# weleen/AGRL.pytorch

Hardware: NVIDIA B200
Metric: MARS-shape tracklets/s (graph head) + query×gallery eval ms at 1/2/4/8 B200 (higher is better)
Workload: dtype fp32 (head GEMMs: fp16 + e4m3 correction planes, distance: fp16x2 planes / 3 products, on tcgen05; fp32 accumulate)

## Files before the change

agrl/pytorch_b200/csrc/gemm_sm100.cuh:

```cuda
#pragma once
#include <cuda.h>
#include <cuda_bf16.h>

#include "common.cuh"

namespace agrl {
namespace gemm {

constexpr int BM = 128, BK = 64;
constexpr int UMMA_K = 16;
constexpr int kTileBytesA = BM * BK * 2;
constexpr int kCtrlWarps = 4;
constexpr int kAccStages = 2;
constexpr int kTmemCols = 512;
constexpr int kEpiPad = 33;
constexpr int kEpiBytes = 4 * 32 * kEpiPad * 4;

template <int P, int BN, bool kSplit, bool kDirect = false, int kChunkKb = 0, bool kPair = false> struct Config {
    static_assert(kChunkKb == 0 || (!kDirect && BN == 128), "chunked accumulation: 128-wide tiles, smem-transposed stores");
    static constexpr int kEpiWarps = (kDirect || kChunkKb > 0) ? 8 : 4;
    static constexpr int kThreads = 32 * (kCtrlWarps + kEpiWarps);
    static_assert(BN == 128 || BN == 256, "tile width");
    static_assert(!kSplit || BN == 128, "two accumulators of 256 columns do not fit twice in TMEM");
    static constexpr int kLoadN = kPair ? BN / 2 : BN;
// ... 39 lines not shown
__device__ __forceinline__ void mbar_wait(uint32_t bar, uint32_t parity) {
    asm volatile(
        "{\n\t"
        ".reg .pred p;\n\t"
        "WAIT_LOOP:\n\t"
        "mbarrier.try_wait.parity.shared::cta.b64 p, [%0], %1;\n\t"
        "@p bra WAIT_DONE;\n\t"
        "bra WAIT_LOOP;\n\t"
        "WAIT_DONE:\n\t"
        "}" ::"r"(bar), "r"(parity) : "memory");
}
__device__ __forceinline__ void tma_load_3d(uint32_t dst, const CUtensorMap *map, uint32_t bar, int c0, int c1, int c2) {
    asm volatile(
        "cp.async.bulk.tensor.3d.shared::cluster.global.mbarrier::complete_tx::bytes [%0], [%1, {%3, %4, %5}], [%2];"
        ::"r"(dst), "l"(reinterpret_cast<uint64_t>(map)), "r"(bar), "r"(c0), "r"(c1), "r"(c2) : "memory");
}
__device__ __forceinline__ void prefetch_tensormap(const CUtensorMap *map) {
    asm volatile("prefetch.tensormap [%0];" ::"l"(reinterpret_cast<uint64_t>(map)) : "memory");
}
__device__ __forceinline__ void tmem_alloc(uint32_t dst_smem, uint32_t ncols) {
    asm volatile("tcgen05.alloc.cta_group::1.sync.aligned.shared::cta.b32 [%0], %1;" ::"r"(dst_smem), "r"(ncols) : "memory");
}
__device__ __forceinline__ void tmem_relinquish() {
    asm volatile("tcgen05.relinquish_alloc_permit.cta_group::1.sync.aligned;" ::: "memory");
}
__device__ __forceinline__ void tmem_dealloc(uint32_t taddr, uint32_t ncols) {
    asm volatile("tcgen05.dealloc.cta_group::1.sync.aligned.b32 %0, %1;" ::"r"(taddr), "r"(ncols) : "memory");
}
__device__ __forceinline__ void tc_fence_before() { asm volatile("tcgen05.fence::before_thread_sync;" ::: "memory"); }
__device__ __forceinline__ void tc_fence_after() { asm volatile("tcgen05.fence::after_thread_sync;" ::: "memory"); }
// ... 597 lines not shown
                  int M, int N, int k_pad, Epi epi) {
    split_gemm_body<P, BN, kSplit, Epi>(map_a, map_b, M, N, k_pad, epi);
}

template <int P, int BN, bool kSplit, class Epi>
__global__ void __cluster_dims__(2, 1, 1) __maxnreg__((Config<P, BN, kSplit, Epi::kDirect, Epi::kChunkKb>::kMaxRegs))
pair_gemm_kernel(const __grid_constant__ CUtensorMap map_a, const __grid_constant__ CUtensorMap map_b,
                 int M, int N, int k_pad, Epi epi) {
    split_gemm_body<P, BN, kSplit, Epi, true>(map_a, map_b, M, N, k_pad, epi);
}

int make_plane_tensor_map(CUtensorMap *map, const void *planes, int64_t rows, int64_t k_pad, int P, int box_rows,
                          int64_t plane_rows);

int make_rows_tensor_map_f32(CUtensorMap *map, const float *x, int64_t batch, int V, int C, int box_channels);

template <int P, int BN, bool kSplit, class Epi>
int launch_pair_gemm(const CUtensorMap &map_a, const CUtensorMap &map_b, int M, int N, int k_pad, const Epi &epi, cudaStream_t st) {
    using Cfg = Config<P, BN, kSplit, Epi::kDirect, Epi::kChunkKb, true>;
    static_assert(!Epi::kDirect || !kSplit, "the direct epilogue reads a single accumulator");
    auto kern = pair_gemm_kernel<P, BN, kSplit, Epi>;
    AGRL_CUDA_TRY(cudaFuncSetAttribute(kern, cudaFuncAttributeMaxDynamicSharedMemorySize, Cfg::kSmemBytes));
    static const int max_pairs = [&] {
        cudaLaunchConfig_t cfg = {};
        cfg.gridDim = dim3(kNumSMs & ~1); cfg.blockDim = dim3(Cfg::kThreads); cfg.dynamicSmemBytes = Cfg::kSmemBytes;
        cudaLaunchAttribute at;
        at.id = cudaLaunchAttributeClusterDimension;
        at.val.clusterDim.x = 2; at.val.clusterDim.y = 1; at.val.clusterDim.z = 1;
        cfg.attrs = &at; cfg.numAttrs = 1;
        int n = 0;
// ... 46 lines not shown
```

agrl/pytorch_b200/csrc/head.cu:

```cuda
#include "gemm_sm100.cuh"

#include <cuda_fp16.h>
#include <cuda_fp8.h>

namespace agrl {

constexpr int kParts = 7;
constexpr int kMaxNodes = 64;
constexpr int kHeadThreads = 256;

static inline int planes_of(int split) { return split == AGRL_SPLIT_FP16_E4M3 ? 2 : split; }
static inline bool scaled_mode(int split) { return split == AGRL_SPLIT_FP16X1 || split == AGRL_SPLIT_FP16_E4M3; }

struct FoldArgs {
    const float *w[AGRL_HEAD_MAX_LAYERS + 2], *b[AGRL_HEAD_MAX_LAYERS + 2];
    const float *mean[AGRL_HEAD_MAX_LAYERS + 2], *var[AGRL_HEAD_MAX_LAYERS + 2];
    float *scale[AGRL_HEAD_MAX_LAYERS + 2], *shift[AGRL_HEAD_MAX_LAYERS + 2];
    int channels;
    float eps;
};

__global__ void fold_bn_kernel(FoldArgs a) {
    const int which = blockIdx.y;
    for (int c = blockIdx.x * blockDim.x + threadIdx.x; c < a.channels; c += gridDim.x * blockDim.x) {
// ... 61 lines not shown
    static __device__ __forceinline__ float cvt(__half v) { return __half2float(v); }
    static __device__ __forceinline__ float4 cvt4(const uint2 &v) {
        const float2 lo = __half22float2(*reinterpret_cast<const __half2 *>(&v.x));
        const float2 hi = __half22float2(*reinterpret_cast<const __half2 *>(&v.y));
        return make_float4(lo.x, lo.y, hi.x, hi.y);
    }
};

template <class T>
struct PoolArgs {
    const T *x41, *x42;
    float *nodes;
    float *out; int64_t ld_out;
    const float *g_scale, *g_shift;
    int S, C, hw;
};

constexpr int kPoolCh = 64;

template <bool kVec, class T>
__global__ void __launch_bounds__(kHeadThreads)
pool_kernel(PoolArgs<T> a) {
    using E = MapElem<T>;
    using Vec4 = typename E::Vec4;
    extern __shared__ float s_nodes[];
    const int b = blockIdx.y, c0 = blockIdx.x * kPoolCh;
    const int warp = threadIdx.x >> 5, lane = threadIdx.x & 31;
    const int grp = lane >> 3, sub = lane & 7;
    const int hw = a.hw, qlen = hw >> 2;
    const float inv_q = 1.0f / static_cast<float>(qlen), inv_h = 1.0f / static_cast<float>(2 * qlen);
// ... 38 lines not shown
            float *dst = s_nodes + (s * kParts) * kPoolCh + warp * 8 + i;
            if (sub == 0) dst[grp * kPoolCh] = v2 * inv_q;
            if (lane == 0) { dst[4 * kPoolCh] = h2 * inv_h; dst[6 * kPoolCh] = w2 * inv_w; }
            if (lane == 16) dst[5 * kPoolCh] = h2 * inv_h;
        }
    }
    if (lane == 0) {
        const float inv_all = 1.0f / (static_cast<float>(a.S) * static_cast<float>(hw));
#pragma unroll
        for (int i = 0; i < 8; ++i) {
            const int c = c0 + warp * 8 + i;
            a.out[static_cast<size_t>(b) * a.ld_out + c] = fmaf(gsum[i] * inv_all, a.g_scale[c], a.g_shift[c]);
        }
    }
    __syncthreads();
    const int V = a.S * kParts;
    float *nodes = a.nodes + static_cast<size_t>(b) * V * a.C + c0;
    for (int i = threadIdx.x; i < V * kPoolCh; i += kHeadThreads) {
        const int v = i / kPoolCh, c = i % kPoolCh;
        nodes[static_cast<size_t>(v) * a.C + c] = s_nodes[i];
    }
}

__device__ __forceinline__ void add4(float4 &a, const float4 &b) { a.x += b.x; a.y += b.y; a.z += b.z; a.w += b.w; }
__device__ __forceinline__ float4 scale4(const float4 &a, float s) { return make_float4(a.x * s, a.y * s, a.z * s, a.w * s); }

template <class T>
__global__ void __launch_bounds__(kHeadThreads)
pool_nhwc_kernel(PoolArgs<T> a) {
    using E = MapElem<T>;
    using Vec4 = typename E::Vec4;
    const int b = blockIdx.y;
    const int c = (blockIdx.x * kHeadThreads + threadIdx.x) * 4;
    if (c >= a.C) return;
    const int hw = a.hw, qlen = hw >> 2, V = a.S * kParts;
// ... 11 lines not shown
#pragma unroll 8
            for (int p = 0; p < qlen; ++p) {
                add4(s1, E::cvt4(__ldcs(reinterpret_cast<const Vec4 *>(a.x41 + base + static_cast<size_t>(p) * a.C))));
                add4(s2, E::cvt4(__ldcs(reinterpret_cast<const Vec4 *>(a.x42 + base + static_cast<size_t>(p) * a.C))));
            }
            add4(g, s1);
            q[k] = s2;
        }
        float4 h0 = q[0], h1 = q[2];
        add4(h0, q[1]); add4(h1, q[3]);
        float4 w = h0;
        add4(w, h1);
        float *row = nodes + static_cast<size_t>(s) * kParts * a.C;
#pragma unroll
        for (int k = 0; k < 4; ++k) *reinterpret_cast<float4 *>(row + static_cast<size_t>(k) * a.C) = scale4(q[k], inv_q);
        *reinterpret_cast<float4 *>(row + 4 * static_cast<size_t>(a.C)) = scale4(h0, inv_h);
        *reinterpret_cast<float4 *>(row + 5 * static_cast<size_t>(a.C)) = scale4(h1, inv_h);
        *reinterpret_cast<float4 *>(row + 6 * static_cast<size_t>(a.C)) = scale4(w, inv_w);
    }
    const float inv_all = 1.0f / (static_cast<float>(a.S) * static_cast<float>(hw));
    const float4 sc = *reinterpret_cast<const float4 *>(a.g_scale + c), sh = *reinterpret_cast<const float4 *>(a.g_shift + c);
    float4 o;
    o.x = fmaf(g.x * inv_all, sc.x, sh.x); o.y = fmaf(g.y * inv_all, sc.y, sh.y);
    o.z = fmaf(g.z * inv_all, sc.z, sh.z); o.w = fmaf(g.w * inv_all, sc.w, sh.w);
    float *dst = a.out + static_cast<size_t>(b) * a.ld_out + c;
    dst[0] = o.x; dst[1] = o.y; dst[2] = o.z; dst[3] = o.w;
}

constexpr int kTpCh = 32;
constexpr int kTpConsumerWarps = 4;
constexpr int kTpThreads = 32 * (1 + kTpConsumerWarps);
template <class T> constexpr int tp_stage_bytes() { return kTpCh * 128 * static_cast<int>(sizeof(T)); }
template <class T> constexpr int tp_default_stages() { return sizeof(T) == 4 ? 4 : 12; }

template <class T>
struct PoolTmaArgs {
    const T *x41, *x42;
    float *nodes;
    float *out; int64_t ld_out;
    const float *g_scale, *g_shift;
    int S, C, stages;
    int unit0, unit1;
    int l2_hint;
};

static size_t pool_tma_smem(int S, int stages, int stage_bytes) {
    const size_t b = static_cast<size_t>(stages) * stage_bytes + 2 * static_cast<size_t>(S) * kParts * kTpCh * sizeof(float) +
                     2 * static_cast<size_t>(stages) * 8;
    return ((b + 127) & ~static_cast<size_t>(127)) + 128;
}

__device__ __forceinline__ void bulk_load_evict_first(uint32_t dst, const void *src, uint32_t bytes, uint32_t bar,
                                                      uint64_t policy) {
    asm volatile(
        "cp.async.bulk.shared::cluster.global.mbarrier::complete_tx::bytes.L2::cache_hint [%0], [%1], %2, [%3], %4;"
        ::"r"(dst), "l"(src), "r"(bytes), "r"(bar), "l"(policy) : "memory");
}

// ... 57 lines not shown
                for (int s = 0; s < S; ++s) {
                    const size_t off = ((static_cast<size_t>(b) * S + s) * C + static_cast<size_t>(cc) * kTpCh) * 128;
#pragma unroll
                    for (int m = 0; m < 2; ++m) {
                        gemm::mbar_wait(bar_empty + 8 * stage, phase ^ 1);
                        const uint32_t full = bar_full + 8 * stage;
                        gemm::mbar_arrive_expect_tx(full, kStageBytes);
                        if (a.l2_hint) bulk_load_evict_first(ring + stage * kStageBytes, (m ? a.x42 : a.x41) + off, kStageBytes, full, policy);
                        else bulk_load(ring + stage * kStageBytes, (m ? a.x42 : a.x41) + off, kStageBytes, full);
                        if (++stage == stages) { stage = 0; phase ^= 1; }
                    }
                }
            }
        }
    } else {
        const int cw = warp - 1, ct = tid - 32;
        const int grp = lane >> 3, sub = lane & 7;
        const float inv_all = 1.0f / (static_cast<float>(S) * 128.0f);
        int stage = 0; uint32_t phase = 0; int it = 0;
        for (int u = first; u < units; u += stride, ++it) {
            const int b = u / chunks, c0 = (u % chunks) * kTpCh;
            float *sn = s_nodes + (it & 1) * V * kTpCh;
            float gsum[8];
#pragma unroll
            for (int i = 0; i < 8; ++i) gsum[i] = 0.f;
            for (int s = 0; s < S; ++s) {
                gemm::mbar_wait(bar_full + 8 * stage, phase);
                {
                    const Vec4 *p = ring_v + stage * kStageVec4 + (cw * 8) * 32 + lane;
#pragma unroll
                    for (int i = 0; i < 8; ++i) {
// ... 26 lines not shown
                    if (grp == 0) dst[6 * kTpCh] = w2 * (1.0f / 128.0f);
                }
                if (++stage == stages) { stage = 0; phase ^= 1; }
            }
            {
                float t = group8_transpose_sum(gsum, sub);
                t += __shfl_xor_sync(0xffffffffu, t, 8);
                t += __shfl_xor_sync(0xffffffffu, t, 16);
                if (grp == 0) {
                    const int c = c0 + cw * 8 + sub;
                    a.out[static_cast<size_t>(b) * a.ld_out + c] = fmaf(t * inv_all, a.g_scale[c], a.g_shift[c]);
                }
            }
            asm volatile("bar.sync 1, %0;" ::"n"(32 * kTpConsumerWarps) : "memory");
            float *nodes = a.nodes + static_cast<size_t>(b) * V * C + c0;
            for (int v = ct >> 5; v < V; v += kTpConsumerWarps) nodes[static_cast<size_t>(v) * C + lane] = sn[v * kTpCh + lane];
        }
    }
}



constexpr int kChunk = 128;
constexpr int kGLd = kMaxNodes + 4;

struct GraphArgs {
    const float *x;
    const float *adj;
    const uint64_t *masks;
    __nv_bfloat16 *y_planes;
    int64_t plane_stride;
// ... 19 lines not shown
        if (adj) return adj[r * V + c];
        const uint64_t hit = ((m0 >> r) & (m0 >> c)) | ((m1 >> r) & (m1 >> c)) | ((m2 >> r) & (m2 >> c));
        return (r != c && (hit & 1ull)) ? 1.0f : 0.0f;
    }
};

constexpr int kTcPlane = 64 * 128;
constexpr int kTcGPlanes = 0;
constexpr int kTcRingOff = 2 * kTcPlane;
constexpr int kTcRingBytes = 8 * kTcPlane;
constexpr int kTcBars = kTcRingOff + kTcRingBytes;
constexpr int kTcRawOff = kTcBars + 256;
constexpr int kTcSmem = kTcRawOff + 1024;
constexpr int kTcThreads = 448;
static_assert((kMaxNodes * kGLd + kMaxNodes) * 4 <= kTcRingBytes, "g[] fits the ring");

__device__ __forceinline__ void fence_proxy_async_smem() { asm volatile("fence.proxy.async.shared::cta;" ::: "memory"); }

template <int P>
__device__ __forceinline__ void split8(const float (&v)[8], uint4 (&out)[P]) {
    float r[8];
#pragma unroll
    for (int i = 0; i < 8; ++i) r[i] = v[i];
#pragma unroll
    for (int p = 0; p < P; ++p) {
        uint32_t w[4];
#pragma unroll
        for (int i = 0; i < 4; ++i) {
            const __nv_bfloat162 b = __floats2bfloat162_rn(r[2 * i], r[2 * i + 1]);
            w[i] = *reinterpret_cast<const uint32_t *>(&b);
// ... 64 lines not shown
            gemm::mbar_init(b_gfull + 8 * i, 8); gemm::mbar_init(b_gdone + 8 * i, 1);
        }
        gemm::fence_barrier_init();
    }
    if (warp == 0) { gemm::tmem_alloc(gemm::smem_u32(tmem_slot), 256); gemm::tmem_relinquish(); }
    if (!a.learn_graph && gram_worker) for (int i = tid; i < kMaxNodes * kGLd; i += kHeadThreads) g[i] = 0.f;
    gemm::tc_fence_before();
    __syncthreads();
    gemm::tc_fence_after();
    const uint32_t tmem = *tmem_slot;
    const bool epi_warp = gram_worker && (warp & 3) < 2;
    const int erow = (warp & 3) * 32 + lane, ehalf = warp >> 2;
    const uint32_t tlane = tmem + (static_cast<uint32_t>((warp & 3) * 32) << 16);
    auto wait_bar = [&](uint32_t bar, int use) { gemm::mbar_wait(bar, static_cast<uint32_t>(use & 1)); };
    const int ref_row = (V > 6) ? 6 : V - 1;
    const int n_gblocks = C / 64;
    if (warp == 0) AGRL_TL(0);
    const int raw_stage = V * 256;
    auto stage_off = [&](int st) { return st < 2 ? kTcRawOff + st * raw_stage : kTcRingOff + 6 * kTcPlane; };
    auto load_raw = [&](int piece, int st) {
        if (lane == 0) {
            const uint32_t full = b_rfull + 8 * st;
            gemm::mbar_arrive_expect_tx(full, static_cast<uint32_t>(raw_stage));
            gemm::tma_load_3d(gemm::smem_u32(smem) + stage_off(st), &map_x, full, piece * 64, 0, b);
        }
    };
    auto gram_uses_of = [&](int st) { return a.learn_graph ? (n_gblocks + 2 - st) / 3 : 0; };
    if (loader && lane == 0) gemm::prefetch_tensormap(&map_x);

    if (a.learn_graph) {
        if (gram_worker) {
            for (int kb = 0; kb < n_gblocks; ++kb) {
                const int buf = kb % 3, use = kb / 3;
                wait_bar(b_rfull + 8 * buf, use);
                if (warp == 0) AGRL_TL(96 + kb);
                if (kb >= 3) wait_bar(b_gdone + 8 * buf, use - 1);
                if (warp == 0) AGRL_TL(192 + kb);
                const float *rs = reinterpret_cast<const float *>(smem + stage_off(buf));
                const float4 *rsrc = reinterpret_cast<const float4 *>(rs + ref_row * 64 + (tid & 7) * 8);
                const float4 rlo = rsrc[0], rhi = rsrc[1];
                unsigned char *dst = ring_p + buf * 2 * kTcPlane;
#pragma unroll
                for (int t = 0; t < 2; ++t) {
                    const int item = tid + kHeadThreads * t, row = item >> 3, slot = item & 7;
                    float c[8];
                    if (row < V) {
                        const float4 *src = reinterpret_cast<const float4 *>(rs + row * 64 + slot * 8);
                        const float4 lo = src[0], hi = src[1];
                        c[0] = __fsub_rn(lo.x, rlo.x); c[1] = __fsub_rn(lo.y, rlo.y); c[2] = __fsub_rn(lo.z, rlo.z); c[3] = __fsub_rn(lo.w, rlo.w);
                        c[4] = __fsub_rn(hi.x, rhi.x); c[5] = __fsub_rn(hi.y, rhi.y); c[6] = __fsub_rn(hi.z, rhi.z); c[7] = __fsub_rn(hi.w, rhi.w);
                    } else {
#pragma unroll
                        for (int i = 0; i < 8; ++i) c[i] = 0.f;
                    }
                    uint4 pl[2];
                    split8<2>(c, pl);
                    const int off = row * 128 + ((slot ^ (row & 7)) << 4);
#pragma unroll
                    for (int p = 0; p < 2; ++p) *reinterpret_cast<uint4 *>(dst + p * kTcPlane + off) = pl[p];
                }
                fence_proxy_async_smem();
                __syncwarp();
                if (lane == 0) { gemm::mbar_arrive(b_gfull + 8 * buf); gemm::mbar_arrive(b_rempty + 8 * buf); }
// ... 73 lines not shown
                m1 = __fdiv_rn(__fdiv_rn(a1, ra) + __fdiv_rn(s1, rs), 2.0f);
            } else if (a.learn_graph) { m0 = __fdiv_rn(s0, rs); m1 = __fdiv_rn(s1, rs); }
            else { m0 = __fdiv_rn(a0, ra); m1 = __fdiv_rn(a1, ra); }
            __syncwarp();
            g[r * kGLd + lane] = (lane < V) ? m0 : 0.f;
            g[r * kGLd + c1] = (c1 < V) ? m1 : 0.f;
        }
    }
    __syncthreads();
    __shared__ float s_scale[2];
    float y_scale = 1.0f;
    if (a.fp16) {
        if (!a.learn_graph) {
            if (worker) {
                for (int r = warp; r < V; r += 12) {
                    const float4 *row = reinterpret_cast<const float4 *>(x + static_cast<size_t>(r) * C);
                    float t = 0.f;
                    for (int i = lane; i < C / 4; i += 32) {
                        const float4 v = __ldg(row + i);
                        t = fmaf(v.x, v.x, t); t = fmaf(v.y, v.y, t); t = fmaf(v.z, v.z, t); t = fmaf(v.w, v.w, t);
                    }
                    t = warp_sum(t);
                    if (lane == 0) sq[r] = t;
                }
            }
            __syncthreads();
        }
        if (warp == 0) {
            float m = fmaxf(lane < V ? sq[lane] : 0.f, lane + 32 < V ? sq[lane + 32] : 0.f);
#pragma unroll
            for (int o = 16; o > 0; o >>= 1) m = fmaxf(m, __shfl_xor_sync(0xffffffffu, m, o));
            float refn = 0.f;
            if (a.learn_graph) {
                const float4 *row = reinterpret_cast<const float4 *>(x + static_cast<size_t>(ref_row) * C);
                for (int i = lane; i < C / 4; i += 32) {
                    const float4 v = __ldg(row + i);
                    refn = fmaf(v.x, v.x, refn); refn = fmaf(v.y, v.y, refn); refn = fmaf(v.z, v.z, refn); refn = fmaf(v.w, v.w, refn);
                }
                refn = warp_sum(refn);
            }
            if (lane == 0) {
                m = (m < 3.0e38f && refn < 3.0e38f) ? sqrtf(m) + sqrtf(refn) : 0.f;
                pow2_scales(m, &s_scale[0], &s_scale[1]);
                a.y_unscale[b] = s_scale[1];
            }
        }
        __syncthreads();
        y_scale = s_scale[0];
    }
    if (a.lowrank) {
        if (worker) {
            const int S4 = (V / kParts) * 4;
            float *gt = a.gt + static_cast<size_t>(b) * V * S4;
            for (int i = tid; i < V * S4; i += 32 * 12) {
                const int r = i / S4, j = i - r * S4, k = j & 3;
                const float *gr = g + r * kGLd + (j >> 2) * kParts;
                gt[i] = fmaf(0.25f, gr[6], fmaf(0.5f, gr[4 + (k >> 1)], gr[k]));
            }
            const int groups = C / 8;
            for (int i = tid; i < S4 * groups; i += 32 * 12) {
                const int qr = i / groups, cg = i - qr * groups;
                const int row = (qr >> 2) * kParts + (qr & 3);
                const float4 *src = reinterpret_cast<const float4 *>(x + static_cast<size_t>(row) * C + cg * 8);
                const float4 lo = __ldg(src), hi = __ldg(src + 1);
                const float v[8] = {lo.x, lo.y, lo.z, lo.w, hi.x, hi.y, hi.z, hi.w};
                __nv_bfloat16 *dst = a.y_planes + (static_cast<size_t>(b) * S4 + qr) * C + cg * 8;
                if (a.fp8) {
// ... 191 lines not shown
    if (warp == 0) AGRL_TL(3);
    gemm::tc_fence_before();
    __syncthreads();
    if (warp == 0) gemm::tmem_dealloc(tmem, 256);
}

constexpr int kMixLdMax = 36;
struct MixArgs {
    const float *x, *z, *gt;
    float *out;
    const float *scale, *shift;
    int V, S4, C;
    float gamma, slope;
};

constexpr int kMixRows = 8;
template <int kMixLd>
__global__ void __launch_bounds__(kHeadThreads, 2)
graph_mix_kernel(MixArgs a) {
    __shared__ __align__(16) float s_gt[kMaxNodes * kMixLd];
    const int b = blockIdx.y, c = (blockIdx.x * kHeadThreads + threadIdx.x) * 2;
    const int V = a.V, S4 = a.S4, C = a.C;
    const float *gt = a.gt + static_cast<size_t>(b) * V * S4;
    for (int i = threadIdx.x; i < V * kMixLd; i += kHeadThreads) {
        const int r = i / kMixLd, k = i - r * kMixLd;
        s_gt[i] = (k < S4) ? gt[r * S4 + k] : 0.f;
    }
    float2 z[kMixLd];
    const float *zc = a.z + static_cast<size_t>(b) * S4 * C + c;
#pragma unroll
    for (int k = 0; k < kMixLd; ++k)
        z[k] = (k < S4) ? __ldg(reinterpret_cast<const float2 *>(zc + static_cast<size_t>(k) * C)) : make_float2(0.f, 0.f);
    const float2 sc = __ldg(reinterpret_cast<const float2 *>(a.scale + c)), sh = __ldg(reinterpret_cast<const float2 *>(a.shift + c));
    const float keep = 1.0f - a.gamma;
    const float *xc = a.x + static_cast<size_t>(b) * V * C + c;
    float *oc = a.out + static_cast<size_t>(b) * V * C + c;
    __syncthreads();
    for (int r0 = 0; r0 < V; r0 += kMixRows) {
        float2 xin[kMixRows];
#pragma unroll
        for (int i = 0; i < kMixRows; ++i)
            xin[i] = (r0 + i < V) ? __ldg(reinterpret_cast<const float2 *>(xc + static_cast<size_t>(r0 + i) * C)) : make_float2(0.f, 0.f);
#pragma unroll
        for (int i = 0; i < kMixRows; ++i) {
            if (r0 + i < V) {
                const float4 *g4 = reinterpret_cast<const float4 *>(s_gt + (r0 + i) * kMixLd);
                float a0 = 0.f, a1 = 0.f;
#pragma unroll
                for (int k4 = 0; k4 < kMixLd / 4; ++k4) {
                    const float4 w = g4[k4];
                    a0 = fmaf(w.x, z[4 * k4 + 0].x, a0); a1 = fmaf(w.x, z[4 * k4 + 0].y, a1);
                    a0 = fmaf(w.y, z[4 * k4 + 1].x, a0); a1 = fmaf(w.y, z[4 * k4 + 1].y, a1);
                    a0 = fmaf(w.z, z[4 * k4 + 2].x, a0); a1 = fmaf(w.z, z[4 * k4 + 2].y, a1);
                    a0 = fmaf(w.w, z[4 * k4 + 3].x, a0); a1 = fmaf(w.w, z[4 * k4 + 3].y, a1);
                }
                float h0 = fmaf(a0, sc.x, sh.x), h1 = fmaf(a1, sc.y, sh.y);
                h0 = h0 >= 0.f ? h0 : h0 * a.slope;
                h1 = h1 >= 0.f ? h1 : h1 * a.slope;
                float2 o;
                o.x = fmaf(a.gamma, h0, keep * xin[i].x);
                o.y = fmaf(a.gamma, h1, keep * xin[i].y);
                *reinterpret_cast<float2 *>(oc + static_cast<size_t>(r0 + i) * C) = o;
            }
        }
    }
}

struct AttnArgs {
    const float *x;
    float *out; int64_t ld_out;
    const float *a_scale, *a_shift;
    int S, C;
    const float *row_sumsq;
    int slots;
};

__global__ void __launch_bounds__(kHeadThreads)
attn_kernel(AttnArgs a) {
// ... 89 lines not shown
    if (!p) return AGRL_E_INVALID;
    if (p->num_layers < 0 || p->num_layers > AGRL_HEAD_MAX_LAYERS) return AGRL_E_INVALID;
    if (p->split != AGRL_SPLIT_BF16X2 && p->split != AGRL_SPLIT_BF16X3 && p->split != AGRL_SPLIT_FP16X1 &&
        p->split != AGRL_SPLIT_FP16_E4M3) return AGRL_E_INVALID;
    if (p->channels < kChunk || p->channels % kChunk != 0) return AGRL_E_UNSUPPORTED;
    if (!p->use_pose && !p->learn_graph) return AGRL_E_INVALID;
    if (p->pool_stages != 0 && (p->pool_stages < 2 || p->pool_stages > 12)) return AGRL_E_INVALID;
    if (p->maps_dtype != AGRL_MAPS_FP32 && p->maps_dtype != AGRL_MAPS_BF16 && p->maps_dtype != AGRL_MAPS_FP16) return AGRL_E_INVALID;
    return AGRL_OK;
}

static int launch_graph(const GraphArgs &ga, int64_t batch, cudaStream_t st) {
    const int smem = kTcSmem + 2 * ga.V * 256;
    AGRL_CUDA_TRY(cudaFuncSetAttribute(graph_kernel_tc, cudaFuncAttributeMaxDynamicSharedMemorySize, kTcSmem + 2 * kMaxNodes * 256));
    CUtensorMap map_x;
    int rc = gemm::make_rows_tensor_map_f32(&map_x, ga.x, batch, ga.V, ga.C, 64);
    if (rc) return rc;
    graph_kernel_tc<<<static_cast<unsigned>(batch), kTcThreads, smem, st>>>(map_x, ga);
    AGRL_LAUNCH_CHECK(st, "graph");
    return AGRL_OK;
}

}

using namespace agrl;

#ifdef AGRL_TIMELINE
extern "C" __attribute__((visibility("default"))) int agrl_timeline_set(long long *buf) {
    return cudaMemcpyToSymbol(g_timeline, &buf, sizeof(buf)) == cudaSuccess ? 0 : -3;
}
#endif
// ... 42 lines not shown
    return AGRL_OK;
}

extern "C" size_t agrl_head_workspace_bytes(const agrl_head_params *p, int64_t batch, int32_t seq_len) {
    if (check_params(p) || batch < 0 || seq_len < 1) return 0;
    return carve_head(p, nullptr, batch, seq_len).bytes;
}

namespace agrl {

template <class T>
static int launch_pool(const agrl_head_params *p, const Prepared &pr, const HeadWorkspace &hwk, const T *x4_1,
                       const T *x4_2, float *out, int64_t ld_out, int64_t b0, int64_t n, int S, int hw, bool tma,
                       cudaStream_t st) {
    const int C = p->channels, V = S * kParts, L = p->num_layers;
    const size_t in_off = static_cast<size_t>(b0) * S * C * hw;
    float *nodes = hwk.x[0] + static_cast<size_t>(b0) * V * C;
    float *o = out + static_cast<size_t>(b0) * ld_out;
    AGRL_LAUNCH_BEGIN(st);
    if (p->maps_nhwc) {
        PoolArgs<T> pa{x4_1 + in_off, x4_2 + in_off, nodes, o, ld_out, pr.scale[L], pr.shift[L], S, C, hw};
        const dim3 grid((C / 4 + kHeadThreads - 1) / kHeadThreads, static_cast<unsigned>(n));
        pool_nhwc_kernel<T><<<grid, kHeadThreads, 0, st>>>(pa);
        AGRL_LAUNCH_CHECK(st, "pool");
        return AGRL_OK;
    }
    if (tma) {
        const int64_t units = n * (C / kTpCh);
        PoolTmaArgs<T> ta{x4_1 + in_off, x4_2 + in_off, nodes, o, ld_out, pr.scale[L], pr.shift[L], S, C,
                          p->pool_stages ? p->pool_stages : tp_default_stages<T>(), 0, static_cast<int>(units),
                          p->pool_no_l2_hint ? 0 : 1};
        const size_t smem = pool_tma_smem(S, ta.stages, tp_stage_bytes<T>());
        AGRL_CUDA_TRY(cudaFuncSetAttribute(pool_tma_kernel<T>, cudaFuncAttributeMaxDynamicSharedMemorySize, static_cast<int>(smem)));
        int64_t grid = static_cast<int64_t>(kNumSMs) * 2;
        if (grid > units) grid = units;
        pool_tma_kernel<T><<<static_cast<unsigned>(grid), kTpThreads, smem, st>>>(ta);
        AGRL_LAUNCH_CHECK(st, "pool");
        return AGRL_OK;
    }
    PoolArgs<T> pa{x4_1 + in_off, x4_2 + in_off, nodes, o, ld_out, pr.scale[L], pr.shift[L], S, C, hw};
    const size_t pool_smem = static_cast<size_t>(S) * kParts * kPoolCh * sizeof(float);
    const dim3 pgrid(C / kPoolCh, static_cast<unsigned>(n));
    const uintptr_t vec_align = 4 * sizeof(T) - 1;
    const bool vec = (hw == 128) && ((reinterpret_cast<uintptr_t>(x4_1) | reinterpret_cast<uintptr_t>(x4_2)) & vec_align) == 0;
    if (vec) pool_kernel<true, T><<<pgrid, kHeadThreads, pool_smem, st>>>(pa);
    else pool_kernel<false, T><<<pgrid, kHeadThreads, pool_smem, st>>>(pa);
    AGRL_LAUNCH_CHECK(st, "pool");
    return AGRL_OK;
}

static int launch_pool_any(const agrl_head_params *p, const Prepared &pr, const HeadWorkspace &hwk, const void *x4_1,
                           const void *x4_2, float *out, int64_t ld_out, int64_t b0, int64_t n, int S, int hw, bool tma,
                           cudaStream_t st) {
    switch (p->maps_dtype) {
        case AGRL_MAPS_BF16:
// ... 191 lines not shown
```

agrl/pytorch_b200/csrc/split.cu:

```cuda
#include "gemm_sm100.cuh"

#include <cuda_fp16.h>
#include <cuda_fp8.h>
#include <mutex>

namespace agrl {
namespace gemm {

constexpr int kSplitThreads = 256;

__global__ void __launch_bounds__(kSplitThreads)
split_planes_kernel(SplitArgs a) {
    __shared__ float s_part[kSplitThreads / 32], s_maxp[kSplitThreads / 32];
    __shared__ float s_inv, s_ps;
    const int64_t row = blockIdx.x;
    const int tid = threadIdx.x;
    const float *src = a.src + row * a.ld;
    const bool vec = ((reinterpret_cast<uintptr_t>(src) & 15u) == 0) && (a.dim % 4 == 0);

    float inv = 1.0f, ps = 1.0f;
    if (a.sumsq != nullptr || a.normalize || a.fp16x2) {
        float s = 0.f, m = 0.f;
        if (vec) {
            const float4 *s4 = reinterpret_cast<const float4 *>(src);
// ... 124 lines not shown
    if (!fn) return AGRL_E_NO_DEVICE;
    const cuuint64_t dims[3] = {static_cast<cuuint64_t>(C), static_cast<cuuint64_t>(V), static_cast<cuuint64_t>(batch)};
    const cuuint64_t strides[2] = {static_cast<cuuint64_t>(C) * 4, static_cast<cuuint64_t>(V) * C * 4};
    const cuuint32_t box[3] = {static_cast<cuuint32_t>(box_channels), static_cast<cuuint32_t>(V), 1};
    const cuuint32_t estr[3] = {1, 1, 1};
    const CUresult r = fn(map, CU_TENSOR_MAP_DATA_TYPE_FLOAT32, 3, const_cast<float *>(x), dims, strides, box, estr,
                          CU_TENSOR_MAP_INTERLEAVE_NONE, CU_TENSOR_MAP_SWIZZLE_NONE,
                          CU_TENSOR_MAP_L2_PROMOTION_L2_256B, CU_TENSOR_MAP_FLOAT_OOB_FILL_NONE);
    if (r != CUDA_SUCCESS) {
        set_cuda_error(cudaErrorInvalidValue, "cuTensorMapEncodeTiled", __FILE__, __LINE__);
        return AGRL_E_CUDA;
    }
    return AGRL_OK;
}

}
}
```

Baseline: 203,200.

## Store only quarter-part nodes and rebuild half/whole parts on the fly

When the low-rank graph path is on, the pooling kernels write only the four quarter-part node rows per frame. The graph and mix kernels rebuild the two half-part rows and the whole-part row as means of the quarters when they need them. The graph kernel loads just the quarter rows through a new 4D TMA map, which cuts the raw staging bytes. It also folds the reference-row norm into the gram-worker loop instead of re-reading it from global memory. This trades pooled-node stores and global reads for a few extra adds, and relies on the half and whole poolings being exact means of the quarters in fp32 rounding order.

```diff
diff --git a/agrl/pytorch_b200/csrc/gemm_sm100.cuh b/agrl/pytorch_b200/csrc/gemm_sm100.cuh
--- a/agrl/pytorch_b200/csrc/gemm_sm100.cuh
+++ b/agrl/pytorch_b200/csrc/gemm_sm100.cuh
@@ -77,6 +77,11 @@
     asm volatile(
         "cp.async.bulk.tensor.3d.shared::cluster.global.mbarrier::complete_tx::bytes [%0], [%1, {%3, %4, %5}], [%2];"
         ::"r"(dst), "l"(reinterpret_cast<uint64_t>(map)), "r"(bar), "r"(c0), "r"(c1), "r"(c2) : "memory");
+}
+__device__ __forceinline__ void tma_load_4d(uint32_t dst, const CUtensorMap *map, uint32_t bar, int c0, int c1, int c2, int c3) {
+    asm volatile(
+        "cp.async.bulk.tensor.4d.shared::cluster.global.mbarrier::complete_tx::bytes [%0], [%1, {%3, %4, %5, %6}], [%2];"
+        ::"r"(dst), "l"(reinterpret_cast<uint64_t>(map)), "r"(bar), "r"(c0), "r"(c1), "r"(c2), "r"(c3) : "memory");
 }
 __device__ __forceinline__ void prefetch_tensormap(const CUtensorMap *map) {
     asm volatile("prefetch.tensormap [%0];" ::"l"(reinterpret_cast<uint64_t>(map)) : "memory");
@@ -704,6 +709,7 @@
                           int64_t plane_rows);
 
 int make_rows_tensor_map_f32(CUtensorMap *map, const float *x, int64_t batch, int V, int C, int box_channels);
+int make_quarter_rows_tensor_map_f32(CUtensorMap *map, const float *x, int64_t batch, int S, int C, int box_channels);
 
 template <int P, int BN, bool kSplit, class Epi>
 int launch_pair_gemm(const CUtensorMap &map_a, const CUtensorMap &map_b, int M, int N, int k_pad, const Epi &epi, cudaStream_t st) {
diff --git a/agrl/pytorch_b200/csrc/head.cu b/agrl/pytorch_b200/csrc/head.cu
--- a/agrl/pytorch_b200/csrc/head.cu
+++ b/agrl/pytorch_b200/csrc/head.cu
@@ -99,6 +99,7 @@
     float *out; int64_t ld_out;
     const float *g_scale, *g_shift;
     int S, C, hw;
+    int quarters_only;
 };
 
 constexpr int kPoolCh = 64;
@@ -167,11 +168,12 @@
         }
     }
     __syncthreads();
-    const int V = a.S * kParts;
+    const int V = a.S * kParts, R = a.quarters_only ? 4 * a.S : V;
     float *nodes = a.nodes + static_cast<size_t>(b) * V * a.C + c0;
-    for (int i = threadIdx.x; i < V * kPoolCh; i += kHeadThreads) {
-        const int v = i / kPoolCh, c = i % kPoolCh;
-        nodes[static_cast<size_t>(v) * a.C + c] = s_nodes[i];
+    for (int i = threadIdx.x; i < R * kPoolCh; i += kHeadThreads) {
+        const int r = i / kPoolCh, c = i % kPoolCh;
+        const int v = a.quarters_only ? (r >> 2) * kParts + (r & 3) : r;
+        nodes[static_cast<size_t>(v) * a.C + c] = s_nodes[v * kPoolCh + c];
     }
 }
 
@@ -213,6 +215,7 @@
         float *row = nodes + static_cast<size_t>(s) * kParts * a.C;
 #pragma unroll
         for (int k = 0; k < 4; ++k) *reinterpret_cast<float4 *>(row + static_cast<size_t>(k) * a.C) = scale4(q[k], inv_q);
+        if (a.quarters_only) continue;
         *reinterpret_cast<float4 *>(row + 4 * static_cast<size_t>(a.C)) = scale4(h0, inv_h);
         *reinterpret_cast<float4 *>(row + 5 * static_cast<size_t>(a.C)) = scale4(h1, inv_h);
         *reinterpret_cast<float4 *>(row + 6 * static_cast<size_t>(a.C)) = scale4(w, inv_w);
@@ -241,6 +244,7 @@
     int S, C, stages;
     int unit0, unit1;
     int l2_hint;
+    int quarters_only;
 };
 
 static size_t pool_tma_smem(int S, int stages, int stage_bytes) {
@@ -328,7 +332,7 @@
             }
         }
     } else {
-        const int cw = warp - 1, ct = tid - 32;
+        const int cw = warp - 1;
         const int grp = lane >> 3, sub = lane & 7;
         const float inv_all = 1.0f / (static_cast<float>(S) * 128.0f);
         int stage = 0; uint32_t phase = 0; int it = 0;
@@ -385,7 +389,8 @@
             }
             asm volatile("bar.sync 1, %0;" ::"n"(32 * kTpConsumerWarps) : "memory");
             float *nodes = a.nodes + static_cast<size_t>(b) * V * C + c0;
-            for (int v = ct >> 5; v < V; v += kTpConsumerWarps) nodes[static_cast<size_t>(v) * C + lane] = sn[v * kTpCh + lane];
+            const int vstep = a.quarters_only ? kParts : kTpConsumerWarps;
+            for (int v = cw; v < V; v += vstep) nodes[static_cast<size_t>(v) * C + lane] = sn[v * kTpCh + lane];
         }
     }
 }
@@ -435,6 +440,14 @@
 constexpr int kTcSmem = kTcRawOff + 1024;
 constexpr int kTcThreads = 448;
 static_assert((kMaxNodes * kGLd + kMaxNodes) * 4 <= kTcRingBytes, "g[] fits the ring");
+
+__device__ __forceinline__ float4 half_mean(const float4 &a, const float4 &b) {
+    return make_float4((a.x + b.x) * 0.5f, (a.y + b.y) * 0.5f, (a.z + b.z) * 0.5f, (a.w + b.w) * 0.5f);
+}
+__device__ __forceinline__ float4 quarter_mean(const float4 &a, const float4 &b, const float4 &c, const float4 &d) {
+    return make_float4(((a.x + b.x) + (c.x + d.x)) * 0.25f, ((a.y + b.y) + (c.y + d.y)) * 0.25f,
+                       ((a.z + b.z) + (c.z + d.z)) * 0.25f, ((a.w + b.w) + (c.w + d.w)) * 0.25f);
+}
 
 __device__ __forceinline__ void fence_proxy_async_smem() { asm volatile("fence.proxy.async.shared::cta;" ::: "memory"); }
 
@@ -529,20 +542,23 @@
     const uint32_t tlane = tmem + (static_cast<uint32_t>((warp & 3) * 32) << 16);
     auto wait_bar = [&](uint32_t bar, int use) { gemm::mbar_wait(bar, static_cast<uint32_t>(use & 1)); };
     const int ref_row = (V > 6) ? 6 : V - 1;
+    const int S4 = (V / kParts) * 4;
     const int n_gblocks = C / 64;
     if (warp == 0) AGRL_TL(0);
-    const int raw_stage = V * 256;
+    const int raw_stage = (a.lowrank ? S4 : V) * 256;
     auto stage_off = [&](int st) { return st < 2 ? kTcRawOff + st * raw_stage : kTcRingOff + 6 * kTcPlane; };
     auto load_raw = [&](int piece, int st) {
         if (lane == 0) {
             const uint32_t full = b_rfull + 8 * st;
             gemm::mbar_arrive_expect_tx(full, static_cast<uint32_t>(raw_stage));
-            gemm::tma_load_3d(gemm::smem_u32(smem) + stage_off(st), &map_x, full, piece * 64, 0, b);
+            if (a.lowrank) gemm::tma_load_4d(gemm::smem_u32(smem) + stage_off(st), &map_x, full, piece * 64, 0, 0, b);
+            else gemm::tma_load_3d(gemm::smem_u32(smem) + stage_off(st), &map_x, full, piece * 64, 0, b);
         }
     };
     auto gram_uses_of = [&](int st) { return a.learn_graph ? (n_gblocks + 2 - st) / 3 : 0; };
     if (loader && lane == 0) gemm::prefetch_tensormap(&map_x);
 
+    float refn_part = 0.f;
     if (a.learn_graph) {
         if (gram_worker) {
             for (int kb = 0; kb < n_gblocks; ++kb) {
@@ -552,16 +568,50 @@
                 if (kb >= 3) wait_bar(b_gdone + 8 * buf, use - 1);
                 if (warp == 0) AGRL_TL(192 + kb);
                 const float *rs = reinterpret_cast<const float *>(smem + stage_off(buf));
-                const float4 *rsrc = reinterpret_cast<const float4 *>(rs + ref_row * 64 + (tid & 7) * 8);
-                const float4 rlo = rsrc[0], rhi = rsrc[1];
+                float4 rlo, rhi;
+                if (a.lowrank) {
+                    const float4 *q = reinterpret_cast<const float4 *>(rs + (lane >> 3) * 64 + (tid & 7) * 8);
+                    rlo = q[0]; rhi = q[1];
+                    float *rv[8] = {&rlo.x, &rlo.y, &rlo.z, &rlo.w, &rhi.x, &rhi.y, &rhi.z, &rhi.w};
+#pragma unroll
+                    for (int i = 0; i < 8; ++i) {
+                        float v = *rv[i];
+                        v += __shfl_xor_sync(0xffffffffu, v, 8);
+                        v += __shfl_xor_sync(0xffffffffu, v, 16);
+                        *rv[i] = v * 0.25f;
+                    }
+                } else {
+                    const float4 *rsrc = reinterpret_cast<const float4 *>(rs + ref_row * 64 + (tid & 7) * 8);
+                    rlo = rsrc[0]; rhi = rsrc[1];
+                }
+                if (tid < 8) {
+                    refn_part = fmaf(rlo.x, rlo.x, refn_part); refn_part = fmaf(rlo.y, rlo.y, refn_part);
+                    refn_part = fmaf(rlo.z, rlo.z, refn_part); refn_part = fmaf(rlo.w, rlo.w, refn_part);
+                    refn_part = fmaf(rhi.x, rhi.x, refn_part); refn_part = fmaf(rhi.y, rhi.y, refn_part);
+                    refn_part = fmaf(rhi.z, rhi.z, refn_part); refn_part = fmaf(rhi.w, rhi.w, refn_part);
+                }
                 unsigned char *dst = ring_p + buf * 2 * kTcPlane;
 #pragma unroll
                 for (int t = 0; t < 2; ++t) {
                     const int item = tid + kHeadThreads * t, row = item >> 3, slot = item & 7;
                     float c[8];
                     if (row < V) {
-                        const float4 *src = reinterpret_cast<const float4 *>(rs + row * 64 + slot * 8);
-                        const float4 lo = src[0], hi = src[1];
+                        float4 lo, hi;
+                        if (a.lowrank) {
+                            const int fs = row / kParts, p = row - fs * kParts;
+                            const float4 *q = reinterpret_cast<const float4 *>(rs + 4 * fs * 64 + slot * 8);
+                            if (p < 4) {
+                                lo = q[16 * p]; hi = q[16 * p + 1];
+                            } else if (p < 6) {
+                                const int h = 32 * (p - 4);
+                                lo = half_mean(q[h], q[h + 16]); hi = half_mean(q[h + 1], q[h + 17]);
+                            } else {
+                                lo = quarter_mean(q[0], q[16], q[32], q[48]); hi = quarter_mean(q[1], q[17], q[33], q[49]);
+                            }
+                        } else {
+                            const float4 *src = reinterpret_cast<const float4 *>(rs + row * 64 + slot * 8);
+                            lo = src[0]; hi = src[1];
+                        }
                         c[0] = __fsub_rn(lo.x, rlo.x); c[1] = __fsub_rn(lo.y, rlo.y); c[2] = __fsub_rn(lo.z, rlo.z); c[3] = __fsub_rn(lo.w, rlo.w);
                         c[4] = __fsub_rn(hi.x, rhi.x); c[5] = __fsub_rn(hi.y, rhi.y); c[6] = __fsub_rn(hi.z, rhi.z); c[7] = __fsub_rn(hi.w, rhi.w);
                     } else {
@@ -665,6 +715,7 @@
         if (!a.learn_graph) {
             if (worker) {
                 for (int r = warp; r < V; r += 12) {
+                    if (a.lowrank && r % kParts >= 4) { if (lane == 0) sq[r] = 0.f; continue; }
                     const float4 *row = reinterpret_cast<const float4 *>(x + static_cast<size_t>(r) * C);
                     float t = 0.f;
                     for (int i = lane; i < C / 4; i += 32) {
@@ -681,15 +732,7 @@
             float m = fmaxf(lane < V ? sq[lane] : 0.f, lane + 32 < V ? sq[lane + 32] : 0.f);
 #pragma unroll
             for (int o = 16; o > 0; o >>= 1) m = fmaxf(m, __shfl_xor_sync(0xffffffffu, m, o));
-            float refn = 0.f;
-            if (a.learn_graph) {
-                const float4 *row = reinterpret_cast<const float4 *>(x + static_cast<size_t>(ref_row) * C);
-                for (int i = lane; i < C / 4; i += 32) {
-                    const float4 v = __ldg(row + i);
-                    refn = fmaf(v.x, v.x, refn); refn = fmaf(v.y, v.y, refn); refn = fmaf(v.z, v.z, refn); refn = fmaf(v.w, v.w, refn);
-                }
-                refn = warp_sum(refn);
-            }
+            const float refn = a.learn_graph ? warp_sum(refn_part) : 0.f;
             if (lane == 0) {
                 m = (m < 3.0e38f && refn < 3.0e38f) ? sqrtf(m) + sqrtf(refn) : 0.f;
                 pow2_scales(m, &s_scale[0], &s_scale[1]);
@@ -701,7 +744,6 @@
     }
     if (a.lowrank) {
         if (worker) {
-            const int S4 = (V / kParts) * 4;
             float *gt = a.gt + static_cast<size_t>(b) * V * S4;
             for (int i = tid; i < V * S4; i += 32 * 12) {
                 const int r = i / S4, j = i - r * S4, k = j & 3;
@@ -923,7 +965,6 @@
     float gamma, slope;
 };
 
-constexpr int kMixRows = 8;
 template <int kMixLd>
 __global__ void __launch_bounds__(kHeadThreads, 2)
 graph_mix_kernel(MixArgs a) {
@@ -945,32 +986,46 @@
     const float *xc = a.x + static_cast<size_t>(b) * V * C + c;
     float *oc = a.out + static_cast<size_t>(b) * V * C + c;
     __syncthreads();
-    for (int r0 = 0; r0 < V; r0 += kMixRows) {
-        float2 xin[kMixRows];
-#pragma unroll
-        for (int i = 0; i < kMixRows; ++i)
-            xin[i] = (r0 + i < V) ? __ldg(reinterpret_cast<const float2 *>(xc + static_cast<size_t>(r0 + i) * C)) : make_float2(0.f, 0.f);
-#pragma unroll
-        for (int i = 0; i < kMixRows; ++i) {
-            if (r0 + i < V) {
-                const float4 *g4 = reinterpret_cast<const float4 *>(s_gt + (r0 + i) * kMixLd);
-                float a0 = 0.f, a1 = 0.f;
-#pragma unroll
-                for (int k4 = 0; k4 < kMixLd / 4; ++k4) {
-                    const float4 w = g4[k4];
-                    a0 = fmaf(w.x, z[4 * k4 + 0].x, a0); a1 = fmaf(w.x, z[4 * k4 + 0].y, a1);
-                    a0 = fmaf(w.y, z[4 * k4 + 1].x, a0); a1 = fmaf(w.y, z[4 * k4 + 1].y, a1);
-                    a0 = fmaf(w.z, z[4 * k4 + 2].x, a0); a1 = fmaf(w.z, z[4 * k4 + 2].y, a1);
-                    a0 = fmaf(w.w, z[4 * k4 + 3].x, a0); a1 = fmaf(w.w, z[4 * k4 + 3].y, a1);
-                }
-                float h0 = fmaf(a0, sc.x, sh.x), h1 = fmaf(a1, sc.y, sh.y);
-                h0 = h0 >= 0.f ? h0 : h0 * a.slope;
-                h1 = h1 >= 0.f ? h1 : h1 * a.slope;
-                float2 o;
-                o.x = fmaf(a.gamma, h0, keep * xin[i].x);
-                o.y = fmaf(a.gamma, h1, keep * xin[i].y);
-                *reinterpret_cast<float2 *>(oc + static_cast<size_t>(r0 + i) * C) = o;
-            }
+    auto load_q = [&](int s, float2 (&q)[4]) {
+#pragma unroll
+        for (int p = 0; p < 4; ++p) q[p] = __ldg(reinterpret_cast<const float2 *>(xc + static_cast<size_t>(s * kParts + p) * C));
+    };
+    float2 qn[4];
+    load_q(0, qn);
+    for (int s = 0; s < V / kParts; ++s) {
+        float2 q[4];
+#pragma unroll
+        for (int p = 0; p < 4; ++p) q[p] = qn[p];
+        if (s + 1 < V / kParts) load_q(s + 1, qn);
+        const int r0 = s * kParts;
+#pragma unroll
+        for (int i = 0; i < kParts; ++i) {
+            float2 xi;
+            if (i < 4) {
+                xi = q[i];
+            } else if (i < 6) {
+                const float2 u = q[2 * (i - 4)], v = q[2 * (i - 4) + 1];
+                xi = make_float2((u.x + v.x) * 0.5f, (u.y + v.y) * 0.5f);
+            } else {
+                xi = make_float2(((q[0].x + q[1].x) + (q[2].x + q[3].x)) * 0.25f, ((q[0].y + q[1].y) + (q[2].y + q[3].y)) * 0.25f);
+            }
+            const float4 *g4 = reinterpret_cast<const float4 *>(s_gt + (r0 + i) * kMixLd);
+            float a0 = 0.f, a1 = 0.f;
+#pragma unroll
+            for (int k4 = 0; k4 < kMixLd / 4; ++k4) {
+                const float4 w = g4[k4];
+                a0 = fmaf(w.x, z[4 * k4 + 0].x, a0); a1 = fmaf(w.x, z[4 * k4 + 0].y, a1);
+                a0 = fmaf(w.y, z[4 * k4 + 1].x, a0); a1 = fmaf(w.y, z[4 * k4 + 1].y, a1);
+                a0 = fmaf(w.z, z[4 * k4 + 2].x, a0); a1 = fmaf(w.z, z[4 * k4 + 2].y, a1);
+                a0 = fmaf(w.w, z[4 * k4 + 3].x, a0); a1 = fmaf(w.w, z[4 * k4 + 3].y, a1);
+            }
+            float h0 = fmaf(a0, sc.x, sh.x), h1 = fmaf(a1, sc.y, sh.y);
+            h0 = h0 >= 0.f ? h0 : h0 * a.slope;
+            h1 = h1 >= 0.f ? h1 : h1 * a.slope;
+            float2 o;
+            o.x = fmaf(a.gamma, h0, keep * xi.x);
+            o.y = fmaf(a.gamma, h1, keep * xi.y);
+            *reinterpret_cast<float2 *>(oc + static_cast<size_t>(r0 + i) * C) = o;
         }
     }
 }
@@ -1090,7 +1145,8 @@
     const int smem = kTcSmem + 2 * ga.V * 256;
     AGRL_CUDA_TRY(cudaFuncSetAttribute(graph_kernel_tc, cudaFuncAttributeMaxDynamicSharedMemorySize, kTcSmem + 2 * kMaxNodes * 256));
     CUtensorMap map_x;
-    int rc = gemm::make_rows_tensor_map_f32(&map_x, ga.x, batch, ga.V, ga.C, 64);
+    int rc = ga.lowrank ? gemm::make_quarter_rows_tensor_map_f32(&map_x, ga.x, batch, ga.V / kParts, ga.C, 64)
+                        : gemm::make_rows_tensor_map_f32(&map_x, ga.x, batch, ga.V, ga.C, 64);
     if (rc) return rc;
     graph_kernel_tc<<<static_cast<unsigned>(batch), kTcThreads, smem, st>>>(map_x, ga);
     AGRL_LAUNCH_CHECK(st, "graph");
@@ -1163,12 +1219,13 @@
                        const T *x4_2, float *out, int64_t ld_out, int64_t b0, int64_t n, int S, int hw, bool tma,
                        cudaStream_t st) {
     const int C = p->channels, V = S * kParts, L = p->num_layers;
+    const int quarters = lowrank_enabled(p, S) ? 1 : 0;
     const size_t in_off = static_cast<size_t>(b0) * S * C * hw;
     float *nodes = hwk.x[0] + static_cast<size_t>(b0) * V * C;
     float *o = out + static_cast<size_t>(b0) * ld_out;
     AGRL_LAUNCH_BEGIN(st);
     if (p->maps_nhwc) {
-        PoolArgs<T> pa{x4_1 + in_off, x4_2 + in_off, nodes, o, ld_out, pr.scale[L], pr.shift[L], S, C, hw};
+        PoolArgs<T> pa{x4_1 + in_off, x4_2 + in_off, nodes, o, ld_out, pr.scale[L], pr.shift[L], S, C, hw, quarters};
         const dim3 grid((C / 4 + kHeadThreads - 1) / kHeadThreads, static_cast<unsigned>(n));
         pool_nhwc_kernel<T><<<grid, kHeadThreads, 0, st>>>(pa);
         AGRL_LAUNCH_CHECK(st, "pool");
@@ -1178,7 +1235,7 @@
         const int64_t units = n * (C / kTpCh);
         PoolTmaArgs<T> ta{x4_1 + in_off, x4_2 + in_off, nodes, o, ld_out, pr.scale[L], pr.shift[L], S, C,
                           p->pool_stages ? p->pool_stages : tp_default_stages<T>(), 0, static_cast<int>(units),
-                          p->pool_no_l2_hint ? 0 : 1};
+                          p->pool_no_l2_hint ? 0 : 1, quarters};
         const size_t smem = pool_tma_smem(S, ta.stages, tp_stage_bytes<T>());
         AGRL_CUDA_TRY(cudaFuncSetAttribute(pool_tma_kernel<T>, cudaFuncAttributeMaxDynamicSharedMemorySize, static_cast<int>(smem)));
         int64_t grid = static_cast<int64_t>(kNumSMs) * 2;
@@ -1187,7 +1244,7 @@
         AGRL_LAUNCH_CHECK(st, "pool");
         return AGRL_OK;
     }
-    PoolArgs<T> pa{x4_1 + in_off, x4_2 + in_off, nodes, o, ld_out, pr.scale[L], pr.shift[L], S, C, hw};
+    PoolArgs<T> pa{x4_1 + in_off, x4_2 + in_off, nodes, o, ld_out, pr.scale[L], pr.shift[L], S, C, hw, quarters};
     const size_t pool_smem = static_cast<size_t>(S) * kParts * kPoolCh * sizeof(float);
     const dim3 pgrid(C / kPoolCh, static_cast<unsigned>(n));
     const uintptr_t vec_align = 4 * sizeof(T) - 1;
diff --git a/agrl/pytorch_b200/csrc/split.cu b/agrl/pytorch_b200/csrc/split.cu
--- a/agrl/pytorch_b200/csrc/split.cu
+++ b/agrl/pytorch_b200/csrc/split.cu
@@ -162,5 +162,23 @@
     return AGRL_OK;
 }
 
+int make_quarter_rows_tensor_map_f32(CUtensorMap *map, const float *x, int64_t batch, int S, int C, int box_channels) {
+    EncodeTiledFn fn = encode_tiled_fn();
+    if (!fn) return AGRL_E_NO_DEVICE;
+    const cuuint64_t row = static_cast<cuuint64_t>(C) * 4;
+    const cuuint64_t dims[4] = {static_cast<cuuint64_t>(C), 4, static_cast<cuuint64_t>(S), static_cast<cuuint64_t>(batch)};
+    const cuuint64_t strides[3] = {row, 7 * row, 7 * static_cast<cuuint64_t>(S) * row};
+    const cuuint32_t box[4] = {static_cast<cuuint32_t>(box_channels), 4, static_cast<cuuint32_t>(S), 1};
+    const cuuint32_t estr[4] = {1, 1, 1, 1};
+    const CUresult r = fn(map, CU_TENSOR_MAP_DATA_TYPE_FLOAT32, 4, const_cast<float *>(x), dims, strides, box, estr,
+                          CU_TENSOR_MAP_INTERLEAVE_NONE, CU_TENSOR_MAP_SWIZZLE_NONE,
+                          CU_TENSOR_MAP_L2_PROMOTION_L2_256B, CU_TENSOR_MAP_FLOAT_OOB_FILL_NONE);
+    if (r != CUDA_SUCCESS) {
+        set_cuda_error(cudaErrorInvalidValue, "cuTensorMapEncodeTiled", __FILE__, __LINE__);
+        return AGRL_E_CUDA;
+    }
+    return AGRL_OK;
+}
+
 }
 }
```

Result: faster. 205,400 (median of 6 runs) (+1.1%).
